# Daniel-Starr/pointcloudhookup

Measured on AMD Instinct MI355X. Metric: Mpts/s ground-filter+tower-cluster, 100 M-pt corridor; % HBM roofline on kNN, higher is better.
Workload: dtype f32 (filter) + f64 (distance predicate)

## Files before the change

### include/pch_hip.h

```cpp
#ifndef PCH_HIP_H
#define PCH_HIP_H

#include <stddef.h>
#include <stdint.h>

#ifdef __cplusplus
extern "C" {
#endif

#define PCH_VERSION 300

#define PCH_OK               0
#define PCH_ERR_ARG         -1
#define PCH_ERR_WORKSPACE   -2
#define PCH_ERR_HIP         -3
#define PCH_ERR_RANGE       -4
#define PCH_ERR_NODEVICE    -5
#define PCH_ERR_TIMEOUT     -6


int         pch_version(void);
const char* pch_last_error(void);
int         pch_device_count(void);

// ... 8 lines not shown
int pch_voxel_canonical_order(const int32_t* idx, const double* mean, const int32_t* count,
                              const int64_t* chunk_offsets, int64_t nchunks, int64_t m,
                              int32_t* out_idx, double* out_mean, int32_t* out_count,
                              int32_t* out_perm ,
                              void* ws, size_t ws_bytes, void* stream);

typedef struct PchLasHeader {
    uint8_t  version_major, version_minor, point_format, reserved0;
    uint16_t header_size, record_length;
    uint32_t offset_to_points, num_vlrs;
    uint64_t point_count;
    double   scales[3], offsets[3], mins[3], maxs[3];
} PchLasHeader;
int    pch_las_read_header(const char* path_host, PchLasHeader* out_host);
size_t pch_las_read_ws_bytes(void);
int    pch_las_read_xyz_i32(const char* path_host, int64_t first, int64_t count, int32_t* out_XYZ,
                            void* ws, size_t ws_bytes, void* stream);
int    pch_las_write_xyz_i32(const char* path_host, const PchLasHeader* hdr_host, const int32_t* XYZ,
                             int64_t n, void* stream);

int pch_las_records_xyz_i32(const uint8_t* records, int64_t n, int32_t record_len,
                            int32_t* out_XYZ, void* stream);

int pch_las_scale_i32_f64(const int32_t* XYZ, int64_t n, const double* scale3_host,
                          const double* offset3_host, double* out_xyz, void* stream);
int pch_las_unscale_f64_i32(const double* xyz, int64_t n, const double* scale3_host,
                            const double* offset3_host, int32_t* out_XYZ, void* stream);

int pch_cast_f64_f32(const double* in, int64_t count, float* out, void* stream);

size_t pch_mean_seq_f32_ws_bytes(int64_t n);
int pch_mean_seq_f32(const float* xyz, int64_t n, float* out_centroid,
                     void* ws, size_t ws_bytes, void* stream);
int pch_mean_seq_partial_f32(const float* xyz, int64_t n, const float* sum_in3, int64_t total_n,
                             float* out3, float* zcol_out, int32_t phase, void* ws, size_t ws_bytes, void* stream);
int pch_mean_seq_serial_f32(const float* xyz, int64_t n, float* out_centroid, void* stream);

size_t pch_percentile_f32_ws_bytes(int64_t n);
int pch_percentile_f32(const float* base, int64_t n, int64_t stride, const float* sub,
                       double q_percent, float* out,
                       void* ws, size_t ws_bytes, void* stream);

int pch_select_hist_f32(const float* base, int64_t n, int64_t stride, int32_t pass, uint32_t prefix,
                        uint32_t* out_hist, unsigned long long* out_nan, void* ws, size_t ws_bytes, void* stream);
int pch_select_min_above_f32(const float* base, int64_t n, int64_t stride, uint32_t key, uint32_t* out_key,
                             void* ws, size_t ws_bytes, void* stream);

size_t pch_filter_gt_ws_bytes(int64_t n);
int pch_filter_gt_f32(const float* raw, int64_t n, const float* centroid3_host, float threshold,
                      float* out_points, int32_t* out_index, int64_t* out_count, float* out_aabb,
                      void* ws, size_t ws_bytes, void* stream);

size_t pch_ground_filter_ws_bytes(int64_t n);
int pch_ground_filter_f32(const float* raw, int64_t n, double pct, float offset,
                          float fallback_offset, int64_t min_keep,
                          float* out_points, int32_t* out_index, float* out_scalars,
                          int64_t* out_count, float* out_aabb,
                          void* ws, size_t ws_bytes, void* stream);

typedef struct PchLasFrame {
    int64_t  centroid[3];
    int64_t  count;
    int64_t  count_at_offset;
    float    base, threshold;
    float    aabb[6];
    uint32_t used_fallback;
// ... 223 lines not shown
```

### pointcloudhookup_amd/_lib.py

```python
from __future__ import annotations

import ctypes as C
import os

_HERE = os.path.dirname(os.path.abspath(__file__))
LIB_PATH = os.path.join(_HERE, "libpch_hip.so")

PCH_OK = 0
ERR_NAMES = {-1: "PCH_ERR_ARG", -2: "PCH_ERR_WORKSPACE", -3: "PCH_ERR_HIP",
             -4: "PCH_ERR_RANGE", -5: "PCH_ERR_NODEVICE", -6: "PCH_ERR_TIMEOUT"}


class PchError(RuntimeError):
    def __init__(self, code, msg):
        super().__init__(f"{ERR_NAMES.get(code, code)}: {msg}")
        self.code = code


_vp, _i64, _i32, _f64, _f32, _sz = C.c_void_p, C.c_int64, C.c_int32, C.c_double, C.c_float, C.c_size_t

_SIGS = {
    "pch_version": (C.c_int, []),
    "pch_last_error": (C.c_char_p, []),
    "pch_device_count": (C.c_int, []),
    "pch_voxel_downsample_ws_bytes": (_sz, [_i64, _i64]),
    "pch_voxel_downsample_f64": (C.c_int, [_vp, _i64, _f64, _i64, _vp, _vp, _vp, _vp, _vp, _vp, _sz, _vp]),
    "pch_voxel_canonical_order_ws_bytes": (_sz, [_i64, _i64]),
    "pch_voxel_canonical_order": (C.c_int, [_vp, _vp, _vp, _vp, _i64, _i64, _vp, _vp, _vp, _vp, _vp, _sz, _vp]),
    "pch_las_read_header": (C.c_int, [C.c_char_p, _vp]),
    "pch_las_read_ws_bytes": (_sz, []),
    "pch_las_read_xyz_i32": (C.c_int, [C.c_char_p, _i64, _i64, _vp, _vp, _sz, _vp]),
    "pch_las_write_xyz_i32": (C.c_int, [C.c_char_p, _vp, _vp, _i64, _vp]),
    "pch_las_records_xyz_i32": (C.c_int, [_vp, _i64, _i32, _vp, _vp]),
    "pch_las_scale_i32_f64": (C.c_int, [_vp, _i64, _vp, _vp, _vp, _vp]),
    "pch_las_unscale_f64_i32": (C.c_int, [_vp, _i64, _vp, _vp, _vp, _vp]),
    "pch_cast_f64_f32": (C.c_int, [_vp, _i64, _vp, _vp]),
    "pch_mean_seq_f32_ws_bytes": (_sz, [_i64]),
    "pch_mean_seq_f32": (C.c_int, [_vp, _i64, _vp, _vp, _sz, _vp]),
    "pch_mean_seq_partial_f32": (C.c_int, [_vp, _i64, _vp, _i64, _vp, _vp, _i32, _vp, _sz, _vp]),
    "pch_mean_seq_serial_f32": (C.c_int, [_vp, _i64, _vp, _vp]),
    "pch_percentile_f32_ws_bytes": (_sz, [_i64]),
    "pch_percentile_f32": (C.c_int, [_vp, _i64, _i64, _vp, _f64, _vp, _vp, _sz, _vp]),
    "pch_select_hist_f32": (C.c_int, [_vp, _i64, _i64, _i32, C.c_uint32, _vp, _vp, _vp, _sz, _vp]),
    "pch_select_min_above_f32": (C.c_int, [_vp, _i64, _i64, C.c_uint32, _vp, _vp, _sz, _vp]),
    "pch_filter_gt_ws_bytes": (_sz, [_i64]),
    "pch_filter_gt_f32": (C.c_int, [_vp, _i64, _vp, _f32, _vp, _vp, _vp, _vp, _vp, _sz, _vp]),
    "pch_ground_filter_ws_bytes": (_sz, [_i64]),
    "pch_ground_filter_f32": (C.c_int, [_vp, _i64, _f64, _f32, _f32, _i64, _vp, _vp, _vp, _vp, _vp,
                                        _vp, _sz, _vp]),
    "pch_ground_filter_las_ws_bytes": (_sz, [_i64]),
    "pch_ground_filter_las_i32": (C.c_int, [_vp, _i64, _vp, _f64, _f32, _f32, _i64, _vp, _vp, _vp, _vp, _sz, _vp]),
    "pch_plane_fit_ws_bytes": (_sz, [_i64, _i32]),
    "pch_plane_fit_f32": (C.c_int, [_vp, _i64, _vp, _vp, _i32, _f64, _f64, _vp, _vp, _vp, _vp, _sz, _vp]),
    "pch_filter_plane_ws_bytes": (_sz, [_i64]),
    "pch_filter_plane_f32": (C.c_int, [_vp, _i64, _vp, _vp, _i32, _f64, _vp, _vp, _vp, _vp, _vp, _sz, _vp]),
    "pch_plane_tiles_fit_ws_bytes": (_sz, [_i64, _i32, _i32]),
    "pch_plane_tiles_fit_f32": (C.c_int, [_vp, _i64, _vp, _vp, _vp, _i32, _i32, _f64, _f64, _vp, _vp, _vp, _vp, _vp,
                                          _sz, _vp]),
    "pch_filter_plane_tiles_ws_bytes": (_sz, [_i64, _i32]),
    "pch_filter_plane_tiles_f32": (C.c_int, [_vp, _i64, _vp, _vp, _vp, _vp, _i32, _f64, _vp, _vp, _vp, _vp, _vp, _sz,
                                             _vp]),
    "pch_dbscan_set_sort_mode": (None, [C.c_int]),
    "pch_first_nonfinite_row_f32": (C.c_int, [_vp, _i64, _vp, _vp]),
    "pch_dbscan_relabel_i32": (C.c_int, [_vp, _i32, _i64, _vp, _vp, _sz, _vp]),
    "pch_dbscan_first_core_rows_i32": (C.c_int, [_i64, _vp, _vp, _sz, _vp]),
    "pch_dbscan_set_pair_counting": (None, [C.c_int]),
    "pch_dbscan_pair_stats": (C.c_int, [_i64, _vp, _vp, _sz, _vp]),
    "pch_dbscan_strip_pairs_i32": (C.c_int, [_i64, _f32, _f32, _i32, _vp, _vp, _vp, _sz, _vp]),
    "pch_dbscan_assign_ws_bytes": (_sz, [_i64]),
    "pch_dbscan_assign_f32": (C.c_int, [_vp, _i64, _vp, _vp, _i64, _vp, _vp, _sz, _vp, _sz, _vp]),
    "pch_dbscan_kdist_ws_bytes": (_sz, [_i64]),
    "pch_dbscan_kdist_f32": (C.c_int, [_vp, _i64, _vp, _vp, _i32, _i64, _vp, _vp, _vp, _sz, _vp, _sz, _vp]),
    "pch_dbscan_knn_ws_bytes": (_sz, [_i64]),
# ... 142 lines not shown
```

### pointcloudhookup_amd/csrc/pch_filter.hip

```cpp
#include "pch_prims.h"
#include "pch_mean.h"
#include "pch_compact.h"
#include "pch_select.h"

namespace pch {

constexpr int SEL_BINS = 4096;
constexpr int SEL_REP0 = 4;
constexpr int SEL_TILE = 4096;

struct SelState {
    unsigned long long rank;
    unsigned long long less;
    uint32_t prefix;
    uint32_t need_next;
    uint32_t v0key;
    uint32_t pad;
};


template <int ROUNDS>
__device__ __forceinline__ void sel_hist_add(uint32_t* h, bool active, uint32_t bin) {
    bool pending = active;
#pragma unroll
// ... 993 lines not shown
                           int64_t* out_count, float* out_aabb, void* ws, size_t ws_bytes, hipStream_t s,
                           GfFollowUp* early) {
    PCH_REQUIRE(n >= 1 && n < (int64_t(1) << 31), "n out of range [1, 2^31) (numpy raises on empty input)");
    PCH_REQUIRE(raw && out_points && out_scalars && out_count && ws, "null buffer");
    PCH_REQUIRE(pct >= 0.0 && pct <= 100.0, "Percentiles must be in the range [0, 100]");
    Arena a(ws, ws_bytes);
    GfWs w;
    gf_plan(a, n, w);
    if (a.overflow) { set_error("workspace too small: need %zu bytes", a.off); return PCH_ERR_WORKSPACE; }
    const int64_t nb = ceil_div(n, GF_TILE);

    w.cand.pct = pct;
    w.cand.add = (offset < fallback_offset ? offset : fallback_offset) - 0.5f;
    bool cand_made = false;
    w.sel.also_zero = reinterpret_cast<uint32_t*>(w.st);
    w.sel.also_words = (int64_t)(w.clear_bytes / 4);
    SideStream& ss = side_stream();
    const bool bracket = ms_makes_cand(n);
    const PctIndex pi = pct_index(n, pct);
    static const bool invalid = getenv("PCH_GF_BRACKET_INVALID") != nullptr;
    const int64_t nblk = ceil_div(n, GF_CBLK);
    const SelBracket r = bracket_ranks(ceil_div(nblk, ms_bracket_stride(nblk)), 1, n, pi);
    w.cand.r_lo = r.r_lo;
    w.cand.r_hi = r.r_hi;
    w.cand.force_invalid = invalid ? 1 : 0;
    const hipStream_t sel_s = ss.ok ? ss.s : s;
    if (ss.ok) {
        PCH_HIP_TRY(hipEventRecord(ss.ev_start, s));
        PCH_HIP_TRY(hipStreamWaitEvent(ss.s, ss.ev_start, 0));
    }
    PCH_LAUNCH("sel_init", sel_init_k, dim3((unsigned)ceil_div(9 * SEL_BINS, 256)), dim3(256), 0, sel_s, w.sel.hist,
               9 * SEL_BINS, w.sel.run, 3, 0ull, 0ull, (unsigned long long)pi.k0, w.sel.br, w.sel.also_zero,
               w.sel.also_words);
    PCH_TRY(mean_seq_launch(raw, n, w.centroid, w.ms, nullptr, s, ss.ok ? ss.ev_fork : nullptr, nullptr, MS_DIVIDE_BY_N,
                            MS_PHASE_BOTH, &w.cand, &cand_made));
    PCH_REQUIRE(!bracket || cand_made, "bracket route without candidate slots");
    if (ss.ok) PCH_HIP_TRY(hipStreamWaitEvent(ss.s, ss.ev_fork, 0));
    if (bracket) {
        PCH_TRY(select_from_summary(raw, n, pct, w.cand, w.sel, sel_s));
    } else {
        const SelGate always = {nullptr, nullptr, nullptr};
        PCH_TRY(select_rounds(raw + 2, n, 3, !pi.same, w.sel.run + 2, w.sel.hist + 6 * SEL_BINS, sel_s, always, n));
    }
    if (ss.ok) {
        PCH_HIP_TRY(hipEventRecord(ss.ev_join, ss.s));
        PCH_HIP_TRY(hipStreamWaitEvent(s, ss.ev_join, 0));
    }
    PCH_TRY(select_lerp(n, w.centroid + 2, pct, offset, fallback_offset, w.sel, s));
    const dim3 grid((unsigned)nb), blk(GF_THREADS);
    const float* tcand = cand_made ? (const float*)w.cand.tcand : (const float*)nullptr;
    const dim3 cgrid((unsigned)ceil_div(nblk, GF_CT_BLKS));
    if (cand_made)
        PCH_LAUNCH("gf_cand", gf_cand_k<0>, cgrid, blk, 0, s, (const float*)w.cand.slots, (const uint32_t*)w.cand.counts,
                   tcand, nblk, (const float*)w.centroid, (const float*)w.sel.scal, w.st, w.status, (long long)min_keep,
                   out_points, out_index);
    PCH_LAUNCH("gf_compact", gf_compact_k<0>, grid, blk, 0, s, raw, n, (const float*)w.centroid,
               (const float*)w.sel.scal, w.st, w.status, (long long)min_keep, out_points, out_index, tcand);
    GfFollowUp fu = {cand_made, cgrid, grid, (const float*)w.cand.slots, (const uint32_t*)w.cand.counts, tcand, nblk, raw, n,
                     (const float*)w.centroid, (const float*)w.sel.scal, w.st, w.status + nb, (long long)min_keep,
                     out_points, out_index, out_scalars, out_count, out_aabb};
    if (early) {
        PCH_LAUNCH("gf_finalize", gf_finalize_k, dim3(1), dim3(64), 0, s, (const GfState*)w.st,
                   (const float*)w.centroid, (const float*)w.sel.scal, out_scalars, out_count, out_aabb);
        *early = fu;
        return PCH_OK;
    }
    return ground_filter_follow_up(fu, s);
}
// ... 14 lines not shown
```

### pointcloudhookup_amd/csrc/pch_mean.h

```cpp
#pragma once
#include "pch_common.h"

namespace pch {

struct MsHdr;
struct MsRec;
struct MsPred;
constexpr int MS_CAND_SLOT = 512;
struct MsBracket {
    uint32_t L, H;
    uint32_t lo_is_min, hi_is_max;
    uint32_t valid[2];
    uint32_t pad[2];
};
struct MsBrRec { uint32_t count_less, nan; };
constexpr int MS_BR_PER = 16;
__host__ __device__ inline int64_t ms_bracket_stride(int64_t ns) {
    const int64_t s = (ns + 1024 * MS_BR_PER - 1) / (1024 * MS_BR_PER);
    return s < 1 ? 1 : s;
}
__device__ __forceinline__ uint32_t sel_key(float v) {
    return (v != v) ? 0xFFFFFFFFu : f32_ordered(v);
}
struct MsCand {
    float*    slots;
    uint32_t* counts;
    float*    tcand;
    float*    zsample;
    double    pct;
    float     add;
    MsBracket* bracket;
    MsBrRec*   brec;
    float*     zseg;
    int64_t    r_lo, r_hi;
    int        force_invalid;
};
struct MsWs {
    MsPred*    pred;
    int*       stats;
    MsRec*     rec;
    MsHdr*     hdr2;
    long long* rows2;
};
void ms_plan(Arena& a, int64_t n, MsWs& w);
constexpr int64_t MS_DIVIDE_BY_N = -1, MS_NO_DIVIDE = -2;
constexpr int MS_PHASE_BOTH = 0, MS_PHASE_TABLES = 1, MS_PHASE_WALK = 2;
bool ms_makes_cand(int64_t n);
int mean_seq_launch(const float* xyz, int64_t n, float* out, MsWs& w, float* zcol, hipStream_t s,
                    hipEvent_t ev_summary = nullptr, const float* sum_in = nullptr, int64_t divide_n = MS_DIVIDE_BY_N,
                    int phase = MS_PHASE_BOTH, const MsCand* cand = nullptr, bool* cand_made = nullptr);

}
```

### pointcloudhookup_amd/csrc/pch_mean.hip

```cpp
#include "pch_mean.h"

namespace pch {

constexpr int MSB       = 1024;
constexpr int MS_PER    = 16;
constexpr int MS_CAND   = 24;
constexpr int MS_ROW2   = 3 * MS_CAND;
constexpr int MS_WAVES  = 4;
constexpr uint32_t MS_NONFINITE = 1u, MS_ALLZERO = 2u;
constexpr uint32_t MS_TIGHT = 4u;
constexpr int MS_FIX_FROM = 11;
constexpr int MS_FIX_LOW  = 6;
constexpr int MS_FIX_MAX  = 16;

struct MsHdr { int emax; uint32_t tie; uint32_t flags; uint32_t mask; };
constexpr uint32_t MS_ALLCAND = (1u << MS_CAND) - 1u;
constexpr int MS_WIN = 4;

struct alignas(128) MsRec {
    MsHdr     h;
    long long A0;
    long long S[MS_CAND];
    uint32_t  fix[MS_CAND];
    uint32_t  pad[18];
// ... 208 lines not shown
    const int l = lane_id(), w = wave_id();
    if (threadIdx.x == 0) carry_sh = sum_in ? (double)sum_in[c] : 0.0;
    __syncthreads();
    for (int64_t r0 = 0; r0 < nb2; r0 += 1024) {
        const int64_t r = r0 + threadIdx.x;
        const double v = r < nb2 ? pred[(int64_t)c * nb2 + r].rowsum : 0.0;
        double incl = v;
#pragma unroll
        for (int o = 1; o < 64; o <<= 1) { const double t = __shfl_up(incl, o, 64); if (l >= o) incl += t; }
        if (l == 63) wsum[w] = incl;
        __syncthreads();
        double woff = 0.0, total = 0.0;
#pragma unroll
        for (int k = 0; k < 16; ++k) { const double t = wsum[k]; woff += k < w ? t : 0.0; total += t; }
        const double carry = carry_sh;
        if (r < nb2) pred[(int64_t)c * nb2 + r].pre = carry + woff + incl - v;
        __syncthreads();
        if (threadIdx.x == 0) carry_sh = carry + total;
        __syncthreads();
    }
}

__device__ __forceinline__ int ms_exp2_floor(double x) {
    return (int)((((unsigned long long)__double_as_longlong(x)) >> 52) & 0x7FFull) - 1023;
}

__global__ __launch_bounds__(64 * MS_WAVES) void ms_summary_k(const float* __restrict__ xyz, int64_t n,
                                                             int64_t nb, MsRec* __restrict__ recs,
                                                             float* __restrict__ zcol,
                                                             const MsPred* __restrict__ pred, int64_t nb2,
                                                             float* __restrict__ cslots, uint32_t* __restrict__ ccounts,
                                                             const float* __restrict__ tcand,
                                                             const MsBracket* __restrict__ brk,
                                                             MsBrRec* __restrict__ brec, float* __restrict__ zseg) {
    __shared__ __attribute__((aligned(16))) float lds[MS_WAVES][MSB * 3];
    __shared__ MsRec stage[MS_WAVES];
    const int64_t blk = (int64_t)blockIdx.x * MS_WAVES + wave_id();
    if (blk >= nb) return;
    const int l = lane_id();
    const int64_t p0 = blk * MSB;
    const int cnt = (int)((n - p0) < MSB ? (n - p0) : MSB);
    float* tile = lds[wave_id()];
    const float* src = xyz + 3 * p0;
    if (cnt == MSB) {
        const float4* s4 = reinterpret_cast<const float4*>(src);
        float4* t4 = reinterpret_cast<float4*>(tile);
#pragma unroll
        for (int i = 0; i < 12; ++i) t4[i * 64 + l] = s4[i * 64 + l];
    } else {
        for (int e = l; e < 3 * MSB; e += 64) tile[e] = e < 3 * cnt ? src[e] : 0.0f;
    }
    __builtin_amdgcn_wave_barrier();
    float zr[MS_PER];
    if (zcol || cslots || brk) {
#pragma unroll
        for (int i = 0; i < MS_PER; ++i) zr[i] = tile[3 * (i * 64 + l) + 2];
    }
    if (zcol) {
#pragma unroll
        for (int i = 0; i < MS_PER; ++i) {
            const int p = i * 64 + l;
            if (p < cnt) zcol[p0 + p] = zr[i];
        }
    }
    if (brk) {
        const bool valid = (brk->valid[0] & brk->valid[1]) != 0u;
        const uint32_t L = valid ? brk->L : 1u, H = valid ? brk->H : 0u;
        uint32_t tally = 0, mask = 0;
#pragma unroll
        for (int i = 0; i < MS_PER; ++i) {
            const bool in = i * 64 + l < cnt;
// ... 439 lines not shown
            s = __uint_as_float(rb);
            r0 = done * (MS_XPART / MS_SEG);
            if (dbg) dbg[0] += done;
            MS_STAMP(3);
        }
        if (r0 < rounds) {
            float a[MS_SEG];
#pragma unroll
            for (int k = 0; k < MS_SEG; ++k) a[k] = X->padded[ms_pad(MS_SEG * l + k)];
            for (int r = r0; r < rounds; ++r) {
                float t = s;
#pragma unroll
                for (int k = 0; k < MS_SEG; ++k) t = t + a[k];
                s = __uint_as_float((uint32_t)__builtin_amdgcn_readlane((int)__float_as_uint(t), r));
            }
            if (dbg) dbg[1] += (rounds - r0) * MS_SEG;
        }
        if (dbg) ++dbg[2];
        __syncthreads();
        MS_STAMP(4);
        ++added;
        if (q == 0 && first_decides) {
            const uint32_t ef = (sb >> 23) & 0xFFu;
            if (((__float_as_uint(s) ^ sb) & 0xFF800000u) == 0 && ef >= 1u && ef <= 254u) break;
        }
    }
    return __float_as_uint(s);
}

constexpr int MS_L2_PITCH = sizeof(MsRec) / 4 + 1;

__global__ __launch_bounds__(256) void ms_level2_k(const MsRec* __restrict__ recs, int64_t nb,
                                                   int64_t nb2, MsHdr* __restrict__ hdr2,
                                                   long long* __restrict__ rows2) {
    __shared__ uint32_t sh[64 * MS_L2_PITCH];
    __shared__ uint32_t tie_sh, miss_sh;
    const int64_t w = blockIdx.x;
    const int c = (int)(w / nb2);
    const int64_t g = w % nb2;
    const int l = lane_id();
    const int64_t bb = g * 64 + l;
    const bool valid = bb < nb;
    {
        const int nchild = (int)((nb - g * 64) < 64 ? (nb - g * 64) : 64);
        const uint4* src = reinterpret_cast<const uint4*>(recs + (int64_t)c * nb + g * 64);
        constexpr int VPR = sizeof(MsRec) / 16;
        uint4 q[VPR / 4];
#pragma unroll
        for (int it = 0; it < VPR / 4; ++it) {
            const int v = it * 256 + (int)threadIdx.x;
            if (v < nchild * VPR) q[it] = src[v];
        }
#pragma unroll
        for (int it = 0; it < VPR / 4; ++it) {
            const int v = it * 256 + (int)threadIdx.x;
            if (v < nchild * VPR) {
                uint32_t* d = sh + (v / VPR) * MS_L2_PITCH + (v % VPR) * 4;
                d[0] = q[it].x; d[1] = q[it].y; d[2] = q[it].z; d[3] = q[it].w;
            }
        }
        if (threadIdx.x == 0) { tie_sh = 0; miss_sh = 0; }
        __syncthreads();
    }
    const uint32_t* rec = sh + l * MS_L2_PITCH;
    auto rec64 = [&](int word) { return (long long)(((unsigned long long)rec[word + 1] << 32) | rec[word]); };
    MsHdr h;
    h.emax = -200; h.tie = 0; h.flags = MS_ALLZERO; h.mask = MS_ALLCAND;
    if (valid) { h.emax = (int)rec[0]; h.tie = rec[1]; h.flags = rec[2]; h.mask = rec[3]; }
    const bool zero = (h.flags & MS_ALLZERO) != 0;
    const int emax2 = wave_reduce_max(zero ? -200 : h.emax);
    const uint32_t nonfinite = __ballot((h.flags & MS_NONFINITE) != 0) ? MS_NONFINITE : 0u;
    const bool allzero = __ballot(!zero) == 0;
// ... 131 lines not shown
            }
        }
        int start = done;
        long long m_cur = (long long)((sb & 0x7FFFFFu) | 0x800000u);
        for (;;) {
            const int f = ms_certify(cls, en, valid, start, count, s_norm, m_cur, sb);
            if (f < 0) { if (start < count) streak = 0; done = count; break; }
            if (f > start) streak = 0;
            {
                const uint32_t mk = (uint32_t)__builtin_amdgcn_readlane((int)h.mask, f);
                const int jf = __builtin_amdgcn_readlane(j, f);
                if (jf >= 0 && jf < MS_CAND && !((mk >> jf) & 1u)) ++n_miss;
            }
            const int extra = streak < count - (f + 1) ? streak : count - (f + 1);
            int added = 0;
            const uint32_t nsb = ms_blocks_exact(xyz, n, c, first + f, 1 + extra, sb, stage, dbg, true, added);
            const bool same = added == 1 && ((nsb ^ sb) & 0xFF800000u) == 0 && s_norm;
            n_exact += added;
            sb = nsb;
            start = f + added;
            done = start;
            if (same) m_cur = (long long)((sb & 0x7FFFFFu) | 0x800000u);
            else {
                streak = streak ? (streak < 16 ? 2 * streak : 32) : 1;
                break;
            }
        }
    }
    return sb;
}

__global__ __launch_bounds__(64 * MS_XW) void ms_walk_k(const float* __restrict__ xyz, int64_t n, MsTables T,
                                                const float* __restrict__ sum_in, int64_t divide_n, int divide,
                                                float* __restrict__ out, int* __restrict__ stats) {
    __shared__ MsExact stage_x;
    MsExact* stage = &stage_x;
    const int c = blockIdx.x;
    const int l = lane_id();
    uint32_t sb = sum_in ? __float_as_uint(sum_in[c]) : 0u;
    int64_t b = 0;
    int n_exact = 0, n_batches = 0, n_desc = 0, n_miss = 0;
    int dbg[3] = {0, 0, 0};
    int streak = 0;
    while (b < T.nb2) {
        ++n_batches;
        const uint32_t ef = (sb >> 23) & 0xFFu;
        if (ef == 255u && (sb & 0x7FFFFFu)) break;
        const bool s_inf = ef == 255u;
        const bool s_norm = ef >= 1u && ef <= 254u;
        const bool s_neg = (sb >> 31) != 0;
        const int E = (int)ef - 127;
        const int64_t bb = b + l;
        const bool valid = bb < T.nb2;
        MsHdr h;
        h.emax = 0; h.tie = 0; h.flags = MS_ALLZERO; h.mask = MS_ALLCAND;
        if (valid) h = T.hdr2[(int64_t)c * T.nb2 + bb];
        int j;
        const int cls = ms_classify(h, valid, s_inf, s_norm, E, j);
        MsEntry en;
        en.n0 = en.n1 = en.lo = en.hi = 0;
        if (cls == 1) {
            en = ms_entry(T.rows2[ms_at(c, j, bb, T.nb2, MS_ROW2)], T.rows2[ms_at(c, MS_CAND + j, bb, T.nb2, MS_ROW2)],
                          T.rows2[ms_at(c, 2 * MS_CAND + j, bb, T.nb2, MS_ROW2)], s_neg);
        }
        int start = 0;
        long long m_cur = (long long)((sb & 0x7FFFFFu) | 0x800000u);
        bool reload = false;
        while (!reload) {
            const int f = ms_certify(cls, en, valid, start, 64, s_norm, m_cur, sb);
            if (f < 0) break;
            ++n_desc;
            const int64_t first = (b + f) * 64;
            const int count = (int)((T.nb - first) < 64 ? (T.nb - first) : 64);
            const uint32_t nsb = ms_walk_children(xyz, n, c, T, first, count, sb, stage, n_exact, streak, n_miss, dbg);
            const bool same = ((nsb ^ sb) & 0xFF800000u) == 0 && s_norm;
            sb = nsb;
            start = f + 1;
            if (same) m_cur = (long long)((sb & 0x7FFFFFu) | 0x800000u);
            else reload = true;
        }
        b += reload ? start : 64;
    }
    if (threadIdx.x == 0) {
        out[c] = divide ? __uint_as_float(sb) / (float)divide_n : __uint_as_float(sb);
        if (stats) {
            stats[4 * c + 0] = n_batches; stats[4 * c + 1] = n_miss;
            stats[4 * c + 2] = n_exact; stats[4 * c + 3] = n_desc;
            stats[16 + 4 * c + 0] = dbg[0]; stats[16 + 4 * c + 1] = dbg[1]; stats[16 + 4 * c + 2] = dbg[2];
#ifdef PCH_MS_STAMPS
            if (c == 2) for (int i = 0; i < 5; ++i) { stats[27 + i] = (int)(ms_stamp_acc[i] >> 6); ms_stamp_acc[i] = 0; }
#endif
        }
    }
}

constexpr int MS_TILE = 4096;

__global__ __launch_bounds__(256) void mean_seq_k(const float* __restrict__ xyz, int64_t n,
                                                  float* __restrict__ out) {
    __shared__ float tile[MS_TILE * 3];
    float s = 0.0f;
    for (int64_t base = 0; base < n; base += MS_TILE) {
        const int cnt = (int)((n - base) < MS_TILE ? (n - base) : MS_TILE);
        const float* src = xyz + 3 * base;
        for (int e = threadIdx.x; e < 3 * cnt; e += 256) tile[e] = src[e];
        __syncthreads();
        if (threadIdx.x < 3) {
            const float* col = tile + threadIdx.x;
            int i = 0;
            for (; i + 8 <= cnt; i += 8) {
                const float a0 = col[3 * (i + 0)], a1 = col[3 * (i + 1)], a2 = col[3 * (i + 2)],
                            a3 = col[3 * (i + 3)], a4 = col[3 * (i + 4)], a5 = col[3 * (i + 5)],
                            a6 = col[3 * (i + 6)], a7 = col[3 * (i + 7)];
                s = s + a0; s = s + a1; s = s + a2; s = s + a3;
                s = s + a4; s = s + a5; s = s + a6; s = s + a7;
            }
            for (; i < cnt; ++i) s = s + col[3 * i];
        }
        __syncthreads();
    }
    if (threadIdx.x < 3) out[threadIdx.x] = s / (float)n;
}

void ms_plan(Arena& a, int64_t n, MsWs& w) {
    const int64_t nb = ceil_div(n > 0 ? n : 1, MSB);
    const int64_t nb2 = ceil_div(nb, 64);
    w.stats = a.take<int>(32);
    w.pred = a.take<MsPred>(3 * nb2);
    w.rec = a.take<MsRec>(3 * nb);
    w.hdr2 = a.take<MsHdr>(3 * nb2);
    w.rows2 = a.take<long long>(3 * nb2 * MS_ROW2);
}

static bool ms_predicts(int64_t n, int phase) {
    static const bool no_predict = getenv("PCH_MEAN_NO_PREDICT") != nullptr;
    return !no_predict && phase == MS_PHASE_BOTH && ceil_div(ceil_div(n, MSB), 64) >= 2;
}
bool ms_makes_cand(int64_t n) {
    static const bool no_cand = getenv("PCH_GF_NO_CAND") != nullptr;
    return n > 0 && !no_cand && ms_predicts(n, MS_PHASE_BOTH);
}

int mean_seq_launch(const float* xyz, int64_t n, float* out, MsWs& w, float* zcol, hipStream_t s,
                    hipEvent_t ev_summary, const float* sum_in, int64_t divide_n, int phase, const MsCand* cand,
                    bool* cand_made) {
    if (cand_made) *cand_made = false;
    const int64_t nb = n > 0 ? ceil_div(n, MSB) : 0;
    const int64_t nb2 = ceil_div(nb, 64);
    if (n > 0 && phase != MS_PHASE_WALK) {
        const MsPred* pred = nullptr;
        bool bracket = false;
        if (ms_predicts(n, phase)) {
            const bool mk = cand && ms_makes_cand(n);
            bracket = mk && cand->bracket;
            MsBrArgs ba;
            memset(&ba, 0, sizeof(ba));
            if (bracket) {
                ba.out = cand->bracket;
                ba.stride = ms_bracket_stride(nb);
                const int64_t ne = ceil_div(nb, ba.stride);
                ba.rank[0] = (uint32_t)cand->r_lo; ba.rank[1] = (uint32_t)cand->r_hi;
                ba.open[0] = cand->r_lo == 0; ba.open[1] = cand->r_hi == ne - 1;
                ba.force_invalid = cand->force_invalid;
            }
            PCH_LAUNCH("mean_sample", ms_sample_k, dim3((unsigned)nb2), dim3(64), 0, s, xyz, n, nb, nb2, w.pred,
                       mk ? cand->zsample : (float*)nullptr);
            PCH_LAUNCH("mean_prefix", ms_prefix_k, dim3(mk ? (bracket ? 6 : 4) : 3), dim3(1024), 0, s, w.pred, nb2, sum_in,
                       mk ? (const float*)cand->zsample : (const float*)nullptr, nb, mk ? cand->pct : 0.0,
                       mk ? cand->add : 0.0f, mk ? cand->tcand : (float*)nullptr, ba);
            pred = w.pred;
            if (mk && cand_made) *cand_made = true;
        }
        const bool emit = cand && cand_made && *cand_made;
        PCH_LAUNCH("mean_summary", ms_summary_k, dim3((unsigned)ceil_div(nb, MS_WAVES)), dim3(64 * MS_WAVES),
                   0, s, xyz, n, nb, w.rec, zcol, pred, nb2,
                   emit ? cand->slots : (float*)nullptr, emit ? cand->counts : (uint32_t*)nullptr,
                   emit ? (const float*)cand->tcand : (const float*)nullptr,
                   bracket ? (const MsBracket*)cand->bracket : (const MsBracket*)nullptr,
                   bracket ? cand->brec : (MsBrRec*)nullptr, bracket ? cand->zseg : (float*)nullptr);
        if (ev_summary) PCH_HIP_TRY(hipEventRecord(ev_summary, s));
        PCH_LAUNCH("mean_level2", ms_level2_k, dim3((unsigned)(3 * nb2)), dim3(256), 0, s,
                   (const MsRec*)w.rec, nb, nb2, w.hdr2, w.rows2);
    }
    if (phase == MS_PHASE_TABLES) return PCH_OK;
    MsTables T;
    T.rec = w.rec; T.nb = nb;
    T.hdr2 = w.hdr2; T.rows2 = w.rows2; T.nb2 = nb2;
    const int divide = divide_n != MS_NO_DIVIDE;
    PCH_LAUNCH("mean_walk", ms_walk_k, dim3(3), dim3(64 * MS_XW), 0, s, xyz, n, T, sum_in,
               divide_n == MS_DIVIDE_BY_N ? n : divide_n, divide, out, w.stats);
    return PCH_OK;
}

}

using namespace pch;

extern "C" size_t pch_mean_seq_f32_ws_bytes(int64_t n) {
    if (n < 0) return 0;
    Arena a;
    MsWs w;
    ms_plan(a, n, w);
    return a.off;
}

extern "C" int pch_mean_seq_f32(const float* xyz, int64_t n, float* out_centroid, void* ws,
                                size_t ws_bytes, void* stream) {
    PCH_DEVICE_GUARD(xyz ? (const void*)xyz : (const void*)out_centroid);
    PCH_REQUIRE(n >= 0 && out_centroid && ws, "bad argument");
    PCH_REQUIRE(n == 0 || xyz, "null input");
    Arena a(ws, ws_bytes);
    MsWs w;
    ms_plan(a, n, w);
    if (a.overflow) { set_error("workspace too small: need %zu bytes", a.off); return PCH_ERR_WORKSPACE; }
    return mean_seq_launch(xyz, n, out_centroid, w, nullptr, (hipStream_t)stream);
}

extern "C" int pch_mean_seq_partial_f32(const float* xyz, int64_t n, const float* sum_in3, int64_t total_n,
                                        float* out3, float* zcol_out, int32_t phase, void* ws, size_t ws_bytes,
                                        void* stream) {
    PCH_DEVICE_GUARD(ws);
    PCH_REQUIRE(n >= 0 && total_n >= 0 && ws && phase >= 0 && phase <= 2, "bad argument");
    PCH_REQUIRE(phase == MS_PHASE_TABLES || out3, "null output");
    PCH_REQUIRE(n == 0 || xyz, "null input");
    Arena a(ws, ws_bytes, phase == MS_PHASE_WALK);
    MsWs w;
    ms_plan(a, n, w);
    if (a.overflow) { set_error("workspace too small: need %zu bytes", a.off); return PCH_ERR_WORKSPACE; }
    return mean_seq_launch(xyz, n, out3, w, zcol_out, (hipStream_t)stream, nullptr, sum_in3,
                           total_n > 0 ? total_n : MS_NO_DIVIDE, phase);
}

extern "C" int pch_mean_seq_serial_f32(const float* xyz, int64_t n, float* out_centroid, void* stream) {
    PCH_DEVICE_GUARD(xyz ? (const void*)xyz : (const void*)out_centroid);
    PCH_REQUIRE(n >= 0 && out_centroid, "bad argument");
    PCH_REQUIRE(n == 0 || xyz, "null input");
    PCH_LAUNCH("mean_seq_serial", mean_seq_k, dim3(1), dim3(256), 0, (hipStream_t)stream, xyz, n, out_centroid);
    return PCH_OK;
}
```

### pointcloudhookup_amd/ops.py

```python
from __future__ import annotations

import threading

import torch

from . import _lib

_tls = threading.local()


def _stream():
    return torch.cuda.current_stream().cuda_stream


def _ptr(t):
    return 0 if t is None else t.data_ptr()


def _need_cuda(t, dtype, name):
    if not isinstance(t, torch.Tensor) or not t.is_cuda:
        raise TypeError(f"{name} must be a CUDA/HIP tensor (no CPU fallback in the product path)")
    if t.dtype != dtype:
        raise TypeError(f"{name} must be {dtype}, got {t.dtype}")
    return t.contiguous()
# ... 886 lines not shown
        raise ValueError(f"d2 must hold at least k = {k} slots per row and one row per count, got {tuple(d2.shape)} "
                         f"for {count.shape[0]} counts")
    full = count >= k
    near = torch.where(full[:, None], d2[:, :k], torch.zeros((), dtype=torch.float64, device=d2.device))
    mean = torch.sqrt(near).sum(dim=1) / float(k)
    return torch.where(full, mean, torch.full((), float("inf"), dtype=torch.float64, device=d2.device))


def check_shape_radius(radius, eps):
    import math
    r = float(radius)
    if not (math.isfinite(r) and r > 0.0):
        raise ValueError(f"radius must be finite and > 0, got {radius!r}")
    if r > float(eps):
        raise ValueError(f"radius {r} exceeds the fit's eps {float(eps)}: fit at the largest radius of interest")
    return r


def shape_features(count, moments):
    count = _need_cuda(count, torch.int32, "count").reshape(-1)
    moments = _need_cuda(moments, torch.float64, "moments").reshape(-1, 9)
    nq = count.numel()
    if moments.shape[0] != nq:
        raise ValueError("moments must hold nine sums per count")
    with torch.cuda.device(count.device):
        out4 = torch.empty((nq, 4), dtype=torch.float64, device=count.device)
        _lib.check(_lib.lib().pch_shape_features_f64(_ptr(count), _ptr(moments), nq, _ptr(out4), _stream()))
    l1, l2, l3, v = out4.unbind(1)
    ok = l1 > 0
    den = torch.where(ok, l1, torch.ones_like(l1))
    zero = torch.zeros_like(l1)
    return dict(l1=l1, l2=l2, l3=l3, verticality=v, linearity=torch.where(ok, (l1 - l2) / den, zero),
                planarity=torch.where(ok, (l2 - l3) / den, zero), scattering=torch.where(ok, l3 / den, zero))


def set_pair_counting(enable):
    _lib.lib().pch_dbscan_set_pair_counting(1 if enable else 0)


def set_dbscan_sort_mode(mode):
    _lib.lib().pch_dbscan_set_sort_mode({"auto": 0, "chunk": 1, "global": 2}[mode])


def first_nonfinite_row(xyz):
    L = _lib.lib()
    xyz = _need_cuda(xyz, torch.float32, "xyz").reshape(-1, 3)
    out = torch.empty((1,), dtype=torch.int64, device=xyz.device)
    with torch.cuda.device(xyz.device):
        _lib.check(L.pch_first_nonfinite_row_f32(_ptr(xyz), xyz.shape[0], _ptr(out), _stream()))
    return int(out.item())


_nf_hint = {}
_tower_clusters_route = 0


def last_tower_clusters_route():
    return _tower_clusters_route


def tower_clusters(raw, eps=8.0, min_samples=80, chunk_size=50000, pct=25.0, offset=3.0,
                   fallback_offset=1.0, min_keep=1000, want_index=False, segment=True, k_cap=65536):
    import ctypes as C
    L = _lib.lib()
    raw = _need_cuda(raw, torch.float32, "raw").reshape(-1, 3)
    n = raw.shape[0]
# ... 904 lines not shown
```

Baseline: 75510.

## Slice sequential mean into row chunks and overlap walk with summary on side stream

Splits the mean summary kernel into K row slices (two by default for large inputs). Level-2 table building and the sequential walk for earlier slices run on a separate non-blocking stream while later slices are still being summarised. Each slice's walk passes its partial sum to the next through scratch slots in the stats buffer. This hides part of the serial walk latency behind summary bandwidth work, at the cost of extra launches, event synchronisation and cross-stream ordering complexity.

```diff
diff --git a/include/pch_hip.h b/include/pch_hip.h
--- a/include/pch_hip.h
+++ b/include/pch_hip.h
@@ -64,6 +64,7 @@
 size_t pch_mean_seq_f32_ws_bytes(int64_t n);
 int pch_mean_seq_f32(const float* xyz, int64_t n, float* out_centroid,
                      void* ws, size_t ws_bytes, void* stream);
+void pch_mean_set_slices(int k);
 int pch_mean_seq_partial_f32(const float* xyz, int64_t n, const float* sum_in3, int64_t total_n,
                              float* out3, float* zcol_out, int32_t phase, void* ws, size_t ws_bytes, void* stream);
 int pch_mean_seq_serial_f32(const float* xyz, int64_t n, float* out_centroid, void* stream);
diff --git a/pointcloudhookup_amd/_lib.py b/pointcloudhookup_amd/_lib.py
--- a/pointcloudhookup_amd/_lib.py
+++ b/pointcloudhookup_amd/_lib.py
@@ -39,6 +39,7 @@
     "pch_mean_seq_f32": (C.c_int, [_vp, _i64, _vp, _vp, _sz, _vp]),
     "pch_mean_seq_partial_f32": (C.c_int, [_vp, _i64, _vp, _i64, _vp, _vp, _i32, _vp, _sz, _vp]),
     "pch_mean_seq_serial_f32": (C.c_int, [_vp, _i64, _vp, _vp]),
+    "pch_mean_set_slices": (None, [C.c_int]),
     "pch_percentile_f32_ws_bytes": (_sz, [_i64]),
     "pch_percentile_f32": (C.c_int, [_vp, _i64, _i64, _vp, _f64, _vp, _vp, _sz, _vp]),
     "pch_select_hist_f32": (C.c_int, [_vp, _i64, _i64, _i32, C.c_uint32, _vp, _vp, _vp, _sz, _vp]),
diff --git a/pointcloudhookup_amd/csrc/pch_filter.hip b/pointcloudhookup_amd/csrc/pch_filter.hip
--- a/pointcloudhookup_amd/csrc/pch_filter.hip
+++ b/pointcloudhookup_amd/csrc/pch_filter.hip
@@ -1049,8 +1049,12 @@
     PCH_LAUNCH("sel_init", sel_init_k, dim3((unsigned)ceil_div(9 * SEL_BINS, 256)), dim3(256), 0, sel_s, w.sel.hist,
                9 * SEL_BINS, w.sel.run, 3, 0ull, 0ull, (unsigned long long)pi.k0, w.sel.br, w.sel.also_zero,
                w.sel.also_words);
-    PCH_TRY(mean_seq_launch(raw, n, w.centroid, w.ms, nullptr, s, ss.ok ? ss.ev_fork : nullptr, nullptr, MS_DIVIDE_BY_N,
-                            MS_PHASE_BOTH, &w.cand, &cand_made));
+    MsLaunch ml;
+    ml.ev_summary = ss.ok ? ss.ev_fork : nullptr;
+    ml.cand = &w.cand;
+    ml.cand_made = &cand_made;
+    ml.may_slice = true;
+    PCH_TRY(mean_seq_launch(raw, n, w.centroid, w.ms, nullptr, s, ml));
     PCH_REQUIRE(!bracket || cand_made, "bracket route without candidate slots");
     if (ss.ok) PCH_HIP_TRY(hipStreamWaitEvent(ss.s, ss.ev_fork, 0));
     if (bracket) {
diff --git a/pointcloudhookup_amd/csrc/pch_mean.h b/pointcloudhookup_amd/csrc/pch_mean.h
--- a/pointcloudhookup_amd/csrc/pch_mean.h
+++ b/pointcloudhookup_amd/csrc/pch_mean.h
@@ -46,8 +46,16 @@
 constexpr int64_t MS_DIVIDE_BY_N = -1, MS_NO_DIVIDE = -2;
 constexpr int MS_PHASE_BOTH = 0, MS_PHASE_TABLES = 1, MS_PHASE_WALK = 2;
 bool ms_makes_cand(int64_t n);
+struct MsLaunch {
+    hipEvent_t    ev_summary = nullptr;
+    const float*  sum_in = nullptr;
+    int64_t       divide_n = MS_DIVIDE_BY_N;
+    int           phase = MS_PHASE_BOTH;
+    const MsCand* cand = nullptr;
+    bool*         cand_made = nullptr;
+    bool          may_slice = false;
+};
 int mean_seq_launch(const float* xyz, int64_t n, float* out, MsWs& w, float* zcol, hipStream_t s,
-                    hipEvent_t ev_summary = nullptr, const float* sum_in = nullptr, int64_t divide_n = MS_DIVIDE_BY_N,
-                    int phase = MS_PHASE_BOTH, const MsCand* cand = nullptr, bool* cand_made = nullptr);
+                    const MsLaunch& opt = MsLaunch());
 
 }
diff --git a/pointcloudhookup_amd/csrc/pch_mean.hip b/pointcloudhookup_amd/csrc/pch_mean.hip
--- a/pointcloudhookup_amd/csrc/pch_mean.hip
+++ b/pointcloudhookup_amd/csrc/pch_mean.hip
@@ -264,11 +264,12 @@
                                                              float* __restrict__ cslots, uint32_t* __restrict__ ccounts,
                                                              const float* __restrict__ tcand,
                                                              const MsBracket* __restrict__ brk,
-                                                             MsBrRec* __restrict__ brec, float* __restrict__ zseg) {
+                                                             MsBrRec* __restrict__ brec, float* __restrict__ zseg,
+                                                             int64_t blk_first, int64_t blk_count) {
     __shared__ __attribute__((aligned(16))) float lds[MS_WAVES][MSB * 3];
     __shared__ MsRec stage[MS_WAVES];
-    const int64_t blk = (int64_t)blockIdx.x * MS_WAVES + wave_id();
-    if (blk >= nb) return;
+    const int64_t blk = blk_first + (int64_t)blockIdx.x * MS_WAVES + wave_id();
+    if (blk >= blk_first + blk_count) return;
     const int l = lane_id();
     const int64_t p0 = blk * MSB;
     const int cnt = (int)((n - p0) < MSB ? (n - p0) : MSB);
@@ -774,12 +775,13 @@
 
 __global__ __launch_bounds__(256) void ms_level2_k(const MsRec* __restrict__ recs, int64_t nb,
                                                    int64_t nb2, MsHdr* __restrict__ hdr2,
-                                                   long long* __restrict__ rows2) {
+                                                   long long* __restrict__ rows2, int64_t row_first,
+                                                   int64_t row_count) {
     __shared__ uint32_t sh[64 * MS_L2_PITCH];
     __shared__ uint32_t tie_sh, miss_sh;
     const int64_t w = blockIdx.x;
-    const int c = (int)(w / nb2);
-    const int64_t g = w % nb2;
+    const int c = (int)(w / row_count);
+    const int64_t g = row_first + w % row_count;
     const int l = lane_id();
     const int64_t bb = g * 64 + l;
     const bool valid = bb < nb;
@@ -977,17 +979,18 @@
 
 __global__ __launch_bounds__(64 * MS_XW) void ms_walk_k(const float* __restrict__ xyz, int64_t n, MsTables T,
                                                 const float* __restrict__ sum_in, int64_t divide_n, int divide,
-                                                float* __restrict__ out, int* __restrict__ stats) {
+                                                float* __restrict__ out, int* __restrict__ stats,
+                                                int64_t row_begin, int64_t row_end, int stats_add) {
     __shared__ MsExact stage_x;
     MsExact* stage = &stage_x;
     const int c = blockIdx.x;
     const int l = lane_id();
     uint32_t sb = sum_in ? __float_as_uint(sum_in[c]) : 0u;
-    int64_t b = 0;
+    int64_t b = row_begin;
     int n_exact = 0, n_batches = 0, n_desc = 0, n_miss = 0;
     int dbg[3] = {0, 0, 0};
     int streak = 0;
-    while (b < T.nb2) {
+    while (b < row_end) {
         ++n_batches;
         const uint32_t ef = (sb >> 23) & 0xFFu;
         if (ef == 255u && (sb & 0x7FFFFFu)) break;
@@ -996,7 +999,7 @@
         const bool s_neg = (sb >> 31) != 0;
         const int E = (int)ef - 127;
         const int64_t bb = b + l;
-        const bool valid = bb < T.nb2;
+        const bool valid = bb < row_end;
         MsHdr h;
         h.emax = 0; h.tie = 0; h.flags = MS_ALLZERO; h.mask = MS_ALLCAND;
         if (valid) h = T.hdr2[(int64_t)c * T.nb2 + bb];
@@ -1029,9 +1032,10 @@
     if (threadIdx.x == 0) {
         out[c] = divide ? __uint_as_float(sb) / (float)divide_n : __uint_as_float(sb);
         if (stats) {
-            stats[4 * c + 0] = n_batches; stats[4 * c + 1] = n_miss;
-            stats[4 * c + 2] = n_exact; stats[4 * c + 3] = n_desc;
-            stats[16 + 4 * c + 0] = dbg[0]; stats[16 + 4 * c + 1] = dbg[1]; stats[16 + 4 * c + 2] = dbg[2];
+            auto put = [&](int i, int v) { stats[i] = stats_add ? stats[i] + v : v; };
+            put(4 * c + 0, n_batches); put(4 * c + 1, n_miss);
+            put(4 * c + 2, n_exact); put(4 * c + 3, n_desc);
+            put(16 + 4 * c + 0, dbg[0]); put(16 + 4 * c + 1, dbg[1]); put(16 + 4 * c + 2, dbg[2]);
 #ifdef PCH_MS_STAMPS
             if (c == 2) for (int i = 0; i < 5; ++i) { stats[27 + i] = (int)(ms_stamp_acc[i] >> 6); ms_stamp_acc[i] = 0; }
 #endif
@@ -1070,7 +1074,7 @@
 void ms_plan(Arena& a, int64_t n, MsWs& w) {
     const int64_t nb = ceil_div(n > 0 ? n : 1, MSB);
     const int64_t nb2 = ceil_div(nb, 64);
-    w.stats = a.take<int>(32);
+    w.stats = a.take<int>(64);
     w.pred = a.take<MsPred>(3 * nb2);
     w.rec = a.take<MsRec>(3 * nb);
     w.hdr2 = a.take<MsHdr>(3 * nb2);
@@ -1086,12 +1090,68 @@
     return n > 0 && !no_cand && ms_predicts(n, MS_PHASE_BOTH);
 }
 
+constexpr int MS_MAX_SLICES = 8;
+constexpr int64_t MS_SLICE_MIN_ROWS = 1024;
+constexpr int MS_AUTO_SLICES = 2;
+static thread_local int g_ms_slices = 0;
+
+struct MsWalkStream { hipStream_t s; hipEvent_t ev_slice[MS_MAX_SLICES]; hipEvent_t ev_walk; bool ok; };
+struct MsWalkStreams {
+    MsWalkStream ws[PCH_MAX_DEVICES];
+    MsWalkStreams() { for (auto& x : ws) { x.s = nullptr; x.ev_walk = nullptr; x.ok = false; for (auto& e : x.ev_slice) e = nullptr; } }
+    ~MsWalkStreams() {
+        if (!may_release_hip_objects()) return;
+        for (auto& x : ws)
+            if (x.ok) {
+                for (auto& e : x.ev_slice) (void)hipEventDestroy(e);
+                (void)hipEventDestroy(x.ev_walk);
+                (void)hipStreamDestroy(x.s);
+            }
+    }
+};
+static MsWalkStream& ms_walk_stream() {
+    static thread_local MsWalkStreams all;
+    MsWalkStream& x = all.ws[current_device_slot()];
+    if (!x.ok && !x.s) {
+        bool ok = hipStreamCreateWithFlags(&x.s, hipStreamNonBlocking) == hipSuccess &&
+                  hipEventCreateWithFlags(&x.ev_walk, hipEventDisableTiming) == hipSuccess;
+        for (auto& e : x.ev_slice) ok = ok && hipEventCreateWithFlags(&e, hipEventDisableTiming) == hipSuccess;
+        x.ok = ok;
+    }
+    return x;
+}
+static int ms_slice_count(int64_t nb2) {
+    int64_t k = g_ms_slices > 0 ? g_ms_slices : (nb2 >= MS_SLICE_MIN_ROWS ? MS_AUTO_SLICES : 1);
+    k = k > MS_MAX_SLICES ? MS_MAX_SLICES : k;
+    k = k > nb2 ? nb2 : k;
+    return k < 1 ? 1 : (int)k;
+}
+
 int mean_seq_launch(const float* xyz, int64_t n, float* out, MsWs& w, float* zcol, hipStream_t s,
-                    hipEvent_t ev_summary, const float* sum_in, int64_t divide_n, int phase, const MsCand* cand,
-                    bool* cand_made) {
+                    const MsLaunch& opt) {
+    const hipEvent_t ev_summary = opt.ev_summary;
+    const float* const sum_in = opt.sum_in;
+    const int64_t divide_n = opt.divide_n;
+    const int phase = opt.phase;
+    const MsCand* const cand = opt.cand;
+    bool* const cand_made = opt.cand_made;
+    const bool may_slice = opt.may_slice;
     if (cand_made) *cand_made = false;
     const int64_t nb = n > 0 ? ceil_div(n, MSB) : 0;
     const int64_t nb2 = ceil_div(nb, 64);
+    int K = 1;
+    MsWalkStream* ws = nullptr;
+    if (may_slice && phase == MS_PHASE_BOTH && !sum_in && n > 0 && ms_slice_count(nb2) > 1) {
+        ws = &ms_walk_stream();
+        if (ws->ok) K = ms_slice_count(nb2);
+    }
+    int64_t row0[MS_MAX_SLICES + 1];
+    for (int k = 0; k <= K; ++k) row0[k] = nb2 * k / K;
+    auto blocks_of = [&](int k, int64_t& first, int64_t& count) {
+        first = row0[k] * 64;
+        const int64_t end = row0[k + 1] * 64 < nb ? row0[k + 1] * 64 : nb;
+        count = end - first;
+    };
     if (n > 0 && phase != MS_PHASE_WALK) {
         const MsPred* pred = nullptr;
         bool bracket = false;
@@ -1117,23 +1177,49 @@
             if (mk && cand_made) *cand_made = true;
         }
         const bool emit = cand && cand_made && *cand_made;
-        PCH_LAUNCH("mean_summary", ms_summary_k, dim3((unsigned)ceil_div(nb, MS_WAVES)), dim3(64 * MS_WAVES),
-                   0, s, xyz, n, nb, w.rec, zcol, pred, nb2,
-                   emit ? cand->slots : (float*)nullptr, emit ? cand->counts : (uint32_t*)nullptr,
-                   emit ? (const float*)cand->tcand : (const float*)nullptr,
-                   bracket ? (const MsBracket*)cand->bracket : (const MsBracket*)nullptr,
-                   bracket ? cand->brec : (MsBrRec*)nullptr, bracket ? cand->zseg : (float*)nullptr);
+        for (int k = 0; k < K; ++k) {
+            int64_t first, count;
+            blocks_of(k, first, count);
+            PCH_LAUNCH("mean_summary", ms_summary_k, dim3((unsigned)ceil_div(count, MS_WAVES)), dim3(64 * MS_WAVES),
+                       0, s, xyz, n, nb, w.rec, zcol, pred, nb2,
+                       emit ? cand->slots : (float*)nullptr, emit ? cand->counts : (uint32_t*)nullptr,
+                       emit ? (const float*)cand->tcand : (const float*)nullptr,
+                       bracket ? (const MsBracket*)cand->bracket : (const MsBracket*)nullptr,
+                       bracket ? cand->brec : (MsBrRec*)nullptr, bracket ? cand->zseg : (float*)nullptr, first, count);
+            if (k + 1 < K) PCH_HIP_TRY(hipEventRecord(ws->ev_slice[k], s));
+        }
         if (ev_summary) PCH_HIP_TRY(hipEventRecord(ev_summary, s));
-        PCH_LAUNCH("mean_level2", ms_level2_k, dim3((unsigned)(3 * nb2)), dim3(256), 0, s,
-                   (const MsRec*)w.rec, nb, nb2, w.hdr2, w.rows2);
-    }
-    if (phase == MS_PHASE_TABLES) return PCH_OK;
+    }
     MsTables T;
     T.rec = w.rec; T.nb = nb;
     T.hdr2 = w.hdr2; T.rows2 = w.rows2; T.nb2 = nb2;
+    const float* carry = sum_in;
+    auto early_slices = [&]() -> int {
+        for (int k = 0; k + 1 < K; ++k) {
+            float* next = reinterpret_cast<float*>(w.stats + 32 + 4 * (k & 1));
+            PCH_HIP_TRY(hipStreamWaitEvent(ws->s, ws->ev_slice[k], 0));
+            PCH_LAUNCH("mean_level2", ms_level2_k, dim3((unsigned)(3 * (row0[k + 1] - row0[k]))), dim3(256), 0, ws->s,
+                       (const MsRec*)w.rec, nb, nb2, w.hdr2, w.rows2, row0[k], row0[k + 1] - row0[k]);
+            PCH_LAUNCH("mean_walk", ms_walk_k, dim3(3), dim3(64 * MS_XW), 0, ws->s, xyz, n, T, carry, (int64_t)0, 0,
+                       next, w.stats, row0[k], row0[k + 1], k > 0 ? 1 : 0);
+            carry = next;
+        }
+        return PCH_OK;
+    };
+    if (K > 1) {
+        const int rc = early_slices();
+        const hipError_t e1 = hipEventRecord(ws->ev_walk, ws->s);
+        const hipError_t e2 = e1 == hipSuccess ? hipStreamWaitEvent(s, ws->ev_walk, 0) : e1;
+        if (rc != PCH_OK) return rc;
+        PCH_HIP_TRY(e2);
+    }
+    if (n > 0 && phase != MS_PHASE_WALK)
+        PCH_LAUNCH("mean_level2", ms_level2_k, dim3((unsigned)(3 * (nb2 - row0[K - 1]))), dim3(256), 0, s,
+                   (const MsRec*)w.rec, nb, nb2, w.hdr2, w.rows2, row0[K - 1], nb2 - row0[K - 1]);
+    if (phase == MS_PHASE_TABLES) return PCH_OK;
     const int divide = divide_n != MS_NO_DIVIDE;
-    PCH_LAUNCH("mean_walk", ms_walk_k, dim3(3), dim3(64 * MS_XW), 0, s, xyz, n, T, sum_in,
-               divide_n == MS_DIVIDE_BY_N ? n : divide_n, divide, out, w.stats);
+    PCH_LAUNCH("mean_walk", ms_walk_k, dim3(3), dim3(64 * MS_XW), 0, s, xyz, n, T, carry,
+               divide_n == MS_DIVIDE_BY_N ? n : divide_n, divide, out, w.stats, row0[K - 1], nb2, K > 1 ? 1 : 0);
     return PCH_OK;
 }
 
@@ -1158,8 +1244,12 @@
     MsWs w;
     ms_plan(a, n, w);
     if (a.overflow) { set_error("workspace too small: need %zu bytes", a.off); return PCH_ERR_WORKSPACE; }
-    return mean_seq_launch(xyz, n, out_centroid, w, nullptr, (hipStream_t)stream);
-}
+    MsLaunch ml;
+    ml.may_slice = true;
+    return mean_seq_launch(xyz, n, out_centroid, w, nullptr, (hipStream_t)stream, ml);
+}
+
+extern "C" void pch_mean_set_slices(int k) { g_ms_slices = k < 0 ? 0 : (k > MS_MAX_SLICES ? MS_MAX_SLICES : k); }
 
 extern "C" int pch_mean_seq_partial_f32(const float* xyz, int64_t n, const float* sum_in3, int64_t total_n,
                                         float* out3, float* zcol_out, int32_t phase, void* ws, size_t ws_bytes,
@@ -1172,8 +1262,11 @@
     MsWs w;
     ms_plan(a, n, w);
     if (a.overflow) { set_error("workspace too small: need %zu bytes", a.off); return PCH_ERR_WORKSPACE; }
-    return mean_seq_launch(xyz, n, out3, w, zcol_out, (hipStream_t)stream, nullptr, sum_in3,
-                           total_n > 0 ? total_n : MS_NO_DIVIDE, phase);
+    MsLaunch ml;
+    ml.sum_in = sum_in3;
+    ml.divide_n = total_n > 0 ? total_n : MS_NO_DIVIDE;
+    ml.phase = phase;
+    return mean_seq_launch(xyz, n, out3, w, zcol_out, (hipStream_t)stream, ml);
 }
 
 extern "C" int pch_mean_seq_serial_f32(const float* xyz, int64_t n, float* out_centroid, void* stream) {
diff --git a/pointcloudhookup_amd/ops.py b/pointcloudhookup_amd/ops.py
--- a/pointcloudhookup_amd/ops.py
+++ b/pointcloudhookup_amd/ops.py
@@ -942,6 +942,10 @@
     zero = torch.zeros_like(l1)
     return dict(l1=l1, l2=l2, l3=l3, verticality=v, linearity=torch.where(ok, (l1 - l2) / den, zero),
                 planarity=torch.where(ok, (l2 - l3) / den, zero), scattering=torch.where(ok, l3 / den, zero))
+
+
+def set_mean_slices(k):
+    _lib.lib().pch_mean_set_slices(int(k))
 
 
 def set_pair_counting(enable):
```

New measurement: 79910 (median of 6 runs). 5.8% higher.
